# mfinzi/depth-estimation

Hardware: AMD Instinct MI355X
Metric: Mpixel-labels/s per CRF mean-field iter (splat+blur+slice) (higher is better)
Workload: dtype f32; 1 GPU; c3: synthetic 2048x1536x256 cost volume, d=5 bilateral features (BASELINE configs[2]); H=1536, W=2048, L=256, d=5, features=synthetic smooth colours sigma_xy=8.0 sigma_c=0.1, n=3145728, M=296893, parallelism=single GPU, launch=eager, arithmetic=default (fp32-rounding-equivalent, ~1e-7 rel), table=reference

## Files before the change

### depth-estimation_amd/csrc/phl_device_utils.h

```cpp
#pragma once
#include <vector>

#include "phl_internal.h"

namespace {

__device__ __forceinline__ void wave_runs(int key, bool active, int *head_lane, int *run_len)
{
    const int lane = threadIdx.x & 63;
    const int prev = __shfl_up(key, 1);
    const bool prev_active = __shfl_up((int)active, 1) != 0;
    const bool head = active && (lane == 0 || !prev_active || prev != key);
    const unsigned long long heads = __ballot(head);
    const unsigned long long act = __ballot(active);
    const unsigned long long below = heads & ((lane == 63) ? ~0ull : ((2ull << lane) - 1ull));
    *head_lane = 63 - __clzll(below ? below : 1ull);
    const unsigned long long above = (lane == 63) ? 0ull : (heads >> (lane + 1));
    const int next_head = above ? lane + 1 + __ffsll((long long)above) - 1 : 64;
    const int last_active = act ? 64 - __clzll(act) : 0;
    *run_len = min(next_head, last_active) - lane;
}

__device__ __forceinline__ int run_atomic_add(int *counters, int key, bool active)
{
// ... 90 lines not shown

__device__ __forceinline__ void tile_prefix_to_lds(const int *__restrict__ tile_sums, int ntiles, int *pre)
{
    const int b4 = threadIdx.x * 4;
    int v[4], s = 0;
#pragma unroll
    for (int i = 0; i < 4; i++) {
        v[i] = (b4 + i) < ntiles ? tile_sums[b4 + i] : 0;
        s += v[i];
    }
    int tot;
    int ex = block_exclusive_scan(s, &tot);
#pragma unroll
    for (int i = 0; i < 4; i++) {
        pre[b4 + i] = ex;
        ex += v[i];
    }
    __syncthreads();
}

__global__ __launch_bounds__(SCAN_T) void k_scan_add_tiles(int *__restrict__ out, const int *__restrict__ tile_sums, int n)
{
    int s = 0;
    for (int i = threadIdx.x; i < (int)blockIdx.x; i += SCAN_T) s += tile_sums[i];
    int add;
    (void)block_exclusive_scan(s, &add);
    if (blockIdx.x == gridDim.x - 1 && threadIdx.x == 0) out[n] = add + tile_sums[blockIdx.x];
    const int base = blockIdx.x * SCAN_TILE + threadIdx.x * SCAN_I;
#pragma unroll
    for (int i = 0; i < SCAN_I; i++)
        if ((base + i) < n) out[base + i] += add;
}

__attribute__((unused)) int exclusive_scan(const int *in, int *out , int n, int *tile_sums, hipStream_t st)
{
    if (n <= 0) {
        PHL_HIP(hipMemsetAsync(out, 0, sizeof(int), st));
        return PHL_OK;
    }
    const int ntiles = (n + SCAN_TILE - 1) / SCAN_TILE;
    hipLaunchKernelGGL(k_scan_tile, dim3(ntiles), dim3(SCAN_T), 0, st, in, out, tile_sums, n);
    if (ntiles <= SCAN_FUSE_TILES) {
        hipLaunchKernelGGL(k_scan_add_tiles, dim3(ntiles), dim3(SCAN_T), 0, st, out, tile_sums, n);
        PHL_HIP(hipGetLastError());
        return PHL_OK;
    }
    hipLaunchKernelGGL(k_scan_sums, dim3(1), dim3(SCAN_T), 0, st, tile_sums, ntiles, out + n);
    hipLaunchKernelGGL(k_scan_add, dim3(ntiles), dim3(SCAN_T), 0, st, out, tile_sums, n);
    PHL_HIP(hipGetLastError());
    return PHL_OK;
}

struct temp_pool {
    std::vector<void *> ptrs;
    char *base = nullptr;
    size_t cap = 0, off = 0, wanted = 0;
    bool have_cache = false;
    temp_pool() { have_cache = phl_scratch_acquire((void **)&base, &cap); }
    ~temp_pool()
    {
        for (void *p : ptrs) (void)hipFree(p);
        if (have_cache) phl_scratch_release(wanted);
    }
    template <typename T>
    hipError_t get(T **out, size_t count)
    {
        const size_t bytes = (((count ? count : 1) * sizeof(T)) + 255) & ~(size_t)255;
        wanted += bytes;
        if (have_cache && off + bytes <= cap) {
            *out = (T *)(base + off);
            off += bytes;
            return hipSuccess;
        }
        void *p = nullptr;
        hipError_t e = hipMalloc(&p, bytes);
        if (e == hipSuccess) ptrs.push_back(p);
        *out = (T *)p;
        return e;
    }
};

constexpr int RS_TILE = 2048;

// ... 131 lines not shown
```

### depth-estimation_amd/csrc/phl_tiles.hip

```cpp
#include <math.h>
#include <stdio.h>
#include <stdlib.h>

#include <map>
#include <mutex>
#include <type_traits>
#include <utility>
#include <vector>

#include "phl_device_utils.h"

namespace {

__global__ __launch_bounds__(256) void k_minmax(const float *__restrict__ ref, int64_t rs, int64_t cs, int64_t n, int d,
                                                float *__restrict__ out )
{
    __shared__ float smin[4][PHL_MAX_D], smax[4][PHL_MAX_D];
    const int lane = threadIdx.x & 63, w = threadIdx.x >> 6;
    float lo[PHL_MAX_D], hi[PHL_MAX_D];
#pragma unroll
    for (int i = 0; i < PHL_MAX_D; i++) { lo[i] = INFINITY; hi[i] = -INFINITY; }
    for (int64_t p = (int64_t)blockIdx.x * blockDim.x + threadIdx.x; p < n; p += (int64_t)gridDim.x * blockDim.x) {
#pragma unroll
        for (int i = 0; i < PHL_MAX_D; i++)
// ... 421 lines not shown
            carry += __shfl(incl, 63);
        }
    }
    __syncthreads();
    const int64_t vbase = vptr ? (int64_t)vptr[c] : (int64_t)c * stride;
    const int vcap = vptr ? SORTN : stride;
    const int64_t ebase = (int64_t)base * dp1;
    if ((int)threadIdx.x < nv) {
        const int v = threadIdx.x;
        const int ni = atomicAdd(&lbin[256 - min(len, 256)], 1);
        newidx[v] = (unsigned short)ni;
        if (ni < vcap) {
            const int64_t sl = vbase + ni;
            slot_vert[sl] = lvid[v];
            seg_rng[sl] = make_int2((int)(ebase + startv[v]), (int)(ebase + startv[v] + len));
        }
    }
    __syncthreads();
#pragma unroll
    for (int u = 0; u < PER; u++) {
        if (vid[u] < 0) continue;
        const int v = id[u], k = kk[u];
        const int pos = (int)startv[v] + (int)cum[v][k >> 5] + __popc(mask[v * 8 + (k >> 5)] & ((1u << (k & 31)) - 1u));
        phl_contrib_t sg;
        sg.pixel = k;
        sg.w = wgt[u];
        seg[ebase + pos] = sg;
        lidx[ebase + i0 + u] = newidx[v];
    }
}

__global__ __launch_bounds__(256) void k_compact_slots(const int *__restrict__ vptr, int nchunks, int stride,
                                                       const int *__restrict__ t_vert, const int2 *__restrict__ t_rng,
                                                       int *__restrict__ slot_vert, int2 *__restrict__ seg_rng)
{
    const int c = blockIdx.x;
    const int b = vptr[c], nv = vptr[c + 1] - b;
    for (int i = threadIdx.x; i < nv; i += 256) {
        slot_vert[b + i] = t_vert[(int64_t)c * stride + i];
        seg_rng[b + i] = t_rng[(int64_t)c * stride + i];
    }
}

__global__ __launch_bounds__(256) void k_count_slots(const int *__restrict__ slot_vert, int S, int *cnt)
{
    const int s = blockIdx.x * blockDim.x + threadIdx.x;
    if (s < S) atomicAdd(&cnt[slot_vert[s]], 1);
}

__global__ __launch_bounds__(256) void k_contrib_and_sole(const int *__restrict__ perm, int *__restrict__ slot_vert, int S,
                                                          const int *__restrict__ vs_ptr, phl_contrib_t *__restrict__ vs,
                                                          int *__restrict__ multi)
{
    const int s = blockIdx.x * blockDim.x + threadIdx.x;
    if (s >= S) return;
    phl_contrib_t c;
    c.pixel = perm[s];
    c.w = 0.f;
    vs[s] = c;
    const int v = slot_vert[s];
    const bool sole = (vs_ptr[v + 1] - vs_ptr[v]) == 1;
    if (sole) slot_vert[s] = v | (int)0x80000000;
    multi[s] = sole ? 0 : 1;
}

__global__ __launch_bounds__(256) void k_append_long(const int *__restrict__ vs_ptr, int M, int long_list, int *__restrict__ vlong,
                                                     int *__restrict__ count)
{
    const int v = blockIdx.x * blockDim.x + threadIdx.x;
    if (v < M && vs_ptr[v + 1] - vs_ptr[v] > long_list) vlong[atomicAdd(count, 1)] = v;
}

__device__ __forceinline__ float4 ld4(const float *p) { return *reinterpret_cast<const float4 *>(p); }
__device__ __forceinline__ void st4(float *p, float4 v) { *reinterpret_cast<float4 *>(p) = v; }
__device__ __forceinline__ float div_c(float t, float c, float rc)
{
    float q = t * rc;
    float rem = __builtin_fmaf(-q, c, t);
    return __builtin_fmaf(rem, rc, q);
}
__device__ __forceinline__ float4 term4(float4 acc, float w, float4 v, float c, float rc)
{
    return make_float4(acc.x + div_c(w * v.x, c, rc), acc.y + div_c(w * v.y, c, rc), acc.z + div_c(w * v.z, c, rc),
                       acc.w + div_c(w * v.w, c, rc));
}
__device__ __forceinline__ float4 fma4(float4 acc, float w, float4 v)
{
    return make_float4(__builtin_fmaf(w, v.x, acc.x), __builtin_fmaf(w, v.y, acc.y), __builtin_fmaf(w, v.z, acc.z),
                       __builtin_fmaf(w, v.w, acc.w));
}

#define PHL_ROW_BCAST(x, K) ((unsigned)__builtin_amdgcn_update_dpp(0, (int)(x), 0x150 + (K), 0xF, 0xF, false))

template <int K0>
__device__ __forceinline__ float4 sum8(float4 acc, const uint2 e, const char *rbase)
{
    float4 q[8];
    unsigned w[8];
#define PHL_E(k) w[k] = PHL_ROW_BCAST(e.y, K0 + k); q[k] = *reinterpret_cast<const float4 *>(rbase + PHL_ROW_BCAST(e.x, K0 + k));
    PHL_E(0) PHL_E(1) PHL_E(2) PHL_E(3) PHL_E(4) PHL_E(5) PHL_E(6) PHL_E(7)
#undef PHL_E
#pragma unroll
    for (int k = 0; k < 8; k++) acc = fma4(acc, __uint_as_float(w[k]), q[k]);
// ... 742 lines not shown
    const int cnt = min(P, n - base);
    const int E = cnt * dp1;
    const int64_t ebase = (int64_t)base * dp1;
    const int vbase = vptr[c], nv = vptr[c + 1] - vbase;
    uint2 *ent = reinterpret_cast<uint2 *>(lds);
    int *pixl = reinterpret_cast<int *>(ent + P * dp1);
    int *vl = pixl + P;
    const int fixed = (P * dp1 * 8 + P * 4 + nv * 4 + 15) & ~15;
    float *rows = reinterpret_cast<float *>(reinterpret_cast<char *>(lds) + fixed);
    const int mode = fixed + (int64_t)nv * (NS * 128) <= lds_bytes ? 8 : (fixed + (int64_t)nv * (NS * 64) <= lds_bytes ? 4 : 0);
    const unsigned pitch_bytes = (unsigned)NS * (mode == 8 ? 128u : 64u);
    for (int k = threadIdx.x; k < cnt; k += TPB) pixl[k] = pix_order[base + k];
    if (mode)
        for (int i = threadIdx.x; i < nv; i += TPB) vl[i] = slot_vert[vbase + i] & 0x7FFFFFFF;
    for (int e = threadIdx.x; e < E; e += TPB) {
        const int k = e / dp1, r = e - k * dp1;
        const int p = pix_order[base + k];
        const unsigned li = lidx[ebase + e];
        ent[e] = make_uint2(mode ? li * pitch_bytes : (unsigned)(slot_vert[vbase + li] & 0x7FFFFFFF),
                            __float_as_uint(replay[(int64_t)p * dp1 + r].w));
    }
    __syncthreads();
    if (mode == 8)
        slice_grad_chunk<NS, 8, false>(vertw, L, cnt, nv, ent, pixl, vl, rows, y, y_rs, ref, ref_rs, ref_cs, grad_ref, accumulate,
                                       wx_out, wx_rs, rcdiv);
    else if (mode == 4)
        slice_grad_chunk<NS, 4, false>(vertw, L, cnt, nv, ent, pixl, vl, rows, y, y_rs, ref, ref_rs, ref_cs, grad_ref, accumulate,
                                       wx_out, wx_rs, rcdiv);
    else
        slice_grad_chunk<NS, 8, true>(vertw, L, cnt, nv, ent, pixl, vl, rows, y, y_rs, ref, ref_rs, ref_cs, grad_ref, accumulate,
                                      wx_out, wx_rs, rcdiv);
}

__global__ __launch_bounds__(256) void k_fill_vs_rows(phl_contrib_t *__restrict__ vs, int S, const int *__restrict__ slot_pidx)
{
    const int e = blockIdx.x * blockDim.x + threadIdx.x;
    if (e < S) vs[e].w = __int_as_float(slot_pidx[vs[e].pixel]);
}

__global__ __launch_bounds__(256) void k_long_keys(const int *__restrict__ vlong, int n, const int *__restrict__ vs_ptr, int kmax,
                                                   int *__restrict__ key)
{
    const int i = blockIdx.x * blockDim.x + threadIdx.x;
    if (i < n) key[i] = kmax - min(vs_ptr[vlong[i] + 1] - vs_ptr[vlong[i]], kmax);
}

__global__ __launch_bounds__(256) void k_gather_i32(const int *__restrict__ src, const int *__restrict__ perm, int n, int *__restrict__ dst)
{
    const int i = blockIdx.x * blockDim.x + threadIdx.x;
    if (i < n) dst[i] = src[perm[i]];
}

__global__ __launch_bounds__(256) void k_first_slot(const int *__restrict__ slot_vert, int S, const int *__restrict__ vs_ptr,
                                                    const phl_contrib_t *__restrict__ vs, int *__restrict__ first)
{
    const int s = blockIdx.x * blockDim.x + threadIdx.x;
    if (s >= S) return;
    const int v = slot_vert[s] & 0x7FFFFFFF;
    first[s] = (vs[vs_ptr[v]].pixel == s) ? 1 : 0;
}

__global__ __launch_bounds__(256) void k_fill_vorder(const int *__restrict__ slot_vert, int S, const int *__restrict__ first,
                                                     const int *__restrict__ rank, int M_local, int M,
                                                     int *__restrict__ vorder)
{
    const int i = blockIdx.x * blockDim.x + threadIdx.x;
    if (i < S && first[i]) vorder[rank[i]] = slot_vert[i] & 0x7FFFFFFF;
    if (i >= M_local && i < M) vorder[i] = i;
}

__global__ __launch_bounds__(256) void k_strip_marks(int *slot_vert, int S)
{
    const int s = blockIdx.x * blockDim.x + threadIdx.x;
    if (s < S) slot_vert[s] &= 0x7FFFFFFF;
}

template <typename F>
inline void dispatch_lprs(int lprs, F &&f)
{
    switch (lprs) {
        case 64: f(std::integral_constant<int, 64>{}); break;
        case 32: f(std::integral_constant<int, 32>{}); break;
        case 16: f(std::integral_constant<int, 16>{}); break;
        case 8: f(std::integral_constant<int, 8>{}); break;
        default: f(std::integral_constant<int, 4>{}); break;
    }
}

int lds_budget()
{
    static int b = [] {
        const char *e = getenv("PHL_TILE_LDS");
        int v = e ? atoi(e) : 80 * 1024;
        return v < 8192 ? 8192 : (v > 160 * 1024 ? 160 * 1024 : v);
    }();
    return b;
}

inline int64_t lds_extra(int P, int dp1, int nv_max) { return (int64_t)P * dp1 * 8 + (int64_t)P * 4 + ((int64_t)nv_max + 2) * 8 + 16 + 256; }

struct tile_cfg {
    int lprs = -1;
    size_t lds = 0;
    int cap = 0;
};
inline int64_t lds_big() { return lds_budget() > 160 * 1024 ? lds_budget() : 160 * 1024; }

// ... 252 lines not shown
}
fork_slot *fork_from(hipStream_t st)
{
    fork_slot *f = fork_acquire();
    if (f && (hipEventRecord(f->fork, st) != hipSuccess || hipStreamWaitEvent(f->s, f->fork, 0) != hipSuccess)) {
        (void)hipGetLastError();
        fork_release(f);
        f = nullptr;
    }
    return f;
}
struct fork_guard {
    fork_slot *f = nullptr;
    ~fork_guard()
    {
        if (!f) return;
        (void)hipStreamSynchronize(f->s);
        fork_release(f);
    }
    hipError_t join(hipStream_t st)
    {
        if (!f) return hipSuccess;
        hipError_t e = hipEventRecord(f->join, f->s);
        if (e == hipSuccess) e = hipStreamWaitEvent(st, f->join, 0);
        if (e == hipSuccess) {
            fork_release(f);
            f = nullptr;
        }
        return e;
    }
};
}

int phl_tiles_link_vertices(phl_lattice *lat, hipStream_t st)
{
    const int M = (int)lat->M, S = (int)lat->S;
    phl_pinned_reset();
    if (lat->vs_ptr) PHL_HIP(phl_dev_free(lat->vs_ptr));
    if (lat->vs) PHL_HIP(phl_dev_free(lat->vs));
    if (lat->slot_pidx) PHL_HIP(phl_dev_free(lat->slot_pidx));
    lat->vs_ptr = nullptr;
    lat->vs = nullptr;
    lat->slot_pidx = nullptr;
    lat->S_multi = 0;
    PHL_HIP(phl_dev_malloc((void **)&lat->vs_ptr, sizeof(int) * ((size_t)M + 1)));
    PHL_HIP(phl_dev_malloc((void **)&lat->vs, sizeof(phl_contrib_t) * ((size_t)S + 1)));
    PHL_HIP(phl_dev_malloc((void **)&lat->slot_pidx, sizeof(int) * ((size_t)S + 1)));
    if (S == 0) {
        PHL_HIP(hipMemsetAsync(lat->vs_ptr, 0, sizeof(int) * ((size_t)M + 1), st));
        PHL_HIP(hipStreamSynchronize(st));
        return PHL_OK;
    }
    temp_pool tmp;
    int *cnt, *multi, *tile_sums, *sperm;
    PHL_HIP(tmp.get(&cnt, (size_t)M + 1));
    PHL_HIP(tmp.get(&multi, (size_t)S + 1));
    PHL_HIP(tmp.get(&tile_sums, (size_t)(S > M ? S : M) / SCAN_TILE + 2));
    PHL_HIP(tmp.get(&sperm, (size_t)S));
    PHL_HIP(hipMemsetAsync(cnt, 0, sizeof(int) * ((size_t)M + 1), st));
    const unsigned gS = (unsigned)((S + 255) / 256);
    hipLaunchKernelGGL(k_strip_marks, dim3(gS), dim3(256), 0, st, lat->slot_vert, S);
    hipLaunchKernelGGL(k_count_slots, dim3(gS), dim3(256), 0, st, lat->slot_vert, S, cnt);
    PHL_HIP(hipGetLastError());
    int rc = exclusive_scan(cnt, lat->vs_ptr, M, tile_sums, st);
    if (rc) return rc;
    rc = stable_sort_perm(lat->slot_vert, S, M, sperm, tmp, st);
    if (rc) return rc;
    hipLaunchKernelGGL(k_contrib_and_sole, dim3(gS), dim3(256), 0, st, sperm, lat->slot_vert, S, lat->vs_ptr, lat->vs, multi);
    PHL_HIP(hipGetLastError());
    rc = exclusive_scan(multi, lat->slot_pidx, S, tile_sums, st);
    if (rc) return rc;
    hipLaunchKernelGGL(k_fill_vs_rows, dim3(gS), dim3(256), 0, st, lat->vs, S, lat->slot_pidx);
    PHL_HIP(hipGetLastError());
    int pageable_counts[2] = {0, 0};
    int *counts = (int *)phl_pinned_alloc(sizeof(int) * 2);
    if (!counts) counts = pageable_counts;
    PHL_HIP(hipMemcpyAsync(&counts[0], lat->slot_pidx + S, sizeof(int), hipMemcpyDeviceToHost, st));
    int n_long = 0;
    if (lat->vlong) PHL_HIP(phl_dev_free(lat->vlong));
    lat->vlong = nullptr;
    lat->n_long = 0;
    {
        int *lcount;
        PHL_HIP(tmp.get(&lcount, 1));
        PHL_HIP(hipMemsetAsync(lcount, 0, sizeof(int), st));
        PHL_HIP(phl_dev_malloc((void **)&lat->vlong, sizeof(int) * ((size_t)M + 1)));
        hipLaunchKernelGGL(k_append_long, dim3((M + 255) / 256), dim3(256), 0, st, lat->vs_ptr, M, LONG_LIST, lat->vlong, lcount);
        PHL_HIP(hipGetLastError());
        PHL_HIP(hipMemcpyAsync(&counts[1], lcount, sizeof(int), hipMemcpyDeviceToHost, st));
    }
    if (lat->vorder) PHL_HIP(phl_dev_free(lat->vorder));
    lat->vorder = nullptr;
    PHL_HIP(hipStreamSynchronize(st));
    const int s_multi = counts[0];
    n_long = counts[1];
    lat->S_multi = s_multi;
    lat->n_long = n_long;
    if (n_long > 64) {
        int *lkey, *lperm, *lsorted;
        PHL_HIP(tmp.get(&lkey, (size_t)n_long));
        PHL_HIP(tmp.get(&lperm, (size_t)n_long));
        PHL_HIP(tmp.get(&lsorted, (size_t)n_long));
        const unsigned gl = (unsigned)((n_long + 255) / 256);
        const int kmax = lat->nchunks + 1;
        hipLaunchKernelGGL(k_long_keys, dim3(gl), dim3(256), 0, st, lat->vlong, n_long, lat->vs_ptr, kmax, lkey);
        PHL_HIP(hipGetLastError());
        rc = stable_sort_perm(lkey, n_long, (int64_t)kmax + 1, lperm, tmp, st);
        if (rc) return rc;
        hipLaunchKernelGGL(k_gather_i32, dim3(gl), dim3(256), 0, st, lat->vlong, lperm, n_long, lsorted);
        PHL_HIP(hipGetLastError());
        PHL_HIP(hipMemcpyAsync(lat->vlong, lsorted, sizeof(int) * (size_t)n_long, hipMemcpyDeviceToDevice, st));
        PHL_HIP(hipStreamSynchronize(st));
    }
    return PHL_OK;
}

namespace {
int tile_pixels(int dp1)
{
    int P = 2048 / dp1;
    if (P > 256) P = 256;
    P &= ~15;
    if (const char *e = getenv("PHL_TILE_P")) {
        const int v = atoi(e) & ~15;
        if (v >= 16 && v <= P) P = v;
    }
    return P;
}

template <typename Pool>
int pixel_order(phl_lattice *lat, const float *ref, int64_t rs, int64_t cs, int P, const float *lo, const float *hi, int *cell,
                int *nca_out, int *ncb_out, Pool &tmp, hipStream_t st)
{
    const int d = lat->d, n = (int)lat->n;
    int da = 0, db = -1;
    for (int i = 1; i < d; i++)
        if (hi[i] - lo[i] > hi[da] - lo[da]) da = i;
    for (int i = 0; i < d; i++)
        if (i != da && (db < 0 || hi[i] - lo[i] > hi[db] - lo[db])) db = i;
    double ra = (double)hi[da] - lo[da], rb = db >= 0 ? (double)hi[db] - lo[db] : 0.0;
    if (!(ra > 0) || !isfinite(ra)) ra = 0;
    if (!(rb > 0) || !isfinite(rb)) { rb = 0; db = -1; }
    int nca = 1, ncb = 1;
    float inv_t = 0.f;
    if (ra > 0 && n > P) {
        double T = rb > 0 ? sqrt((double)P * ra * rb / n) : (double)P * ra / n;
        if (T > 0 && isfinite(T)) {
// ... 181 lines not shown
    constexpr int SLOT_STRIDE = 384;
    int *t_vert;
    int2 *t_rng;
    PHL_HIP(tmp.get(&t_vert, (size_t)nchunks * SLOT_STRIDE));
    PHL_HIP(tmp.get(&t_rng, (size_t)nchunks * SLOT_STRIDE));
    PHL_HIP(phl_dev_malloc((void **)&lat->seg, sizeof(phl_contrib_t) * (size_t)N));
    PHL_HIP(phl_dev_malloc((void **)&lat->lidx, sizeof(unsigned short) * (size_t)N));
    static const bool use_masks = !(getenv("PHL_CHUNK_MASKS") && atoi(getenv("PHL_CHUNK_MASKS")) == 0);
    if (use_masks) {
        PHL_CHUNK_MASKS(lat->pix_order, n, P, dp1, lat->replay, nv, (const int *)nullptr, SLOT_STRIDE, t_vert, t_rng, lat->seg,
                        lat->lidx)
    } else {
        PHL_CHUNK_SORT(true, lat->pix_order, n, P, dp1, lat->replay, nv, (const int *)nullptr, SLOT_STRIDE, t_vert, t_rng,
                       lat->seg, lat->lidx, (const int *)nullptr, 0)
    }
    PHL_HIP(hipGetLastError());
    rc = exclusive_scan(nv, lat->chunk_vptr, nchunks, tile_sums, st);
    if (rc) return rc;
    std::vector<int> nv_pageable, by_nv_pageable;
    int *nv_host = (int *)phl_pinned_alloc(sizeof(int) * (size_t)nchunks);
    int *by_nv = (int *)phl_pinned_alloc(sizeof(int) * (size_t)nchunks);
    if (!nv_host) { nv_pageable.resize((size_t)nchunks); nv_host = nv_pageable.data(); }
    if (!by_nv) { by_nv_pageable.resize((size_t)nchunks); by_nv = by_nv_pageable.data(); }
    PHL_HIP(hipMemcpyAsync(nv_host, nv, sizeof(int) * (size_t)nchunks, hipMemcpyDeviceToHost, st));
    PHL_HIP(hipStreamSynchronize(st));
    int nv_max = 0;
    for (int c = 0; c < nchunks; c++) {
        const int v = nv_host[c];
        S += v;
        if (v > nv_max) nv_max = v;
    }
    lat->S = S;
    lat->nv_max = nv_max;
    {
        lat->nv_cum = (int *)malloc(sizeof(int) * ((size_t)nv_max + 2));
        if (!lat->nv_cum) { phl_set_error("phl_tiles_build: out of host memory"); return PHL_ERR_HIP; }
        std::vector<int> start((size_t)nv_max + 2, 0);
        for (int c = 0; c < nchunks; c++) start[(size_t)(nv_max - nv_host[c]) + 1]++;
        for (int b = 0; b <= nv_max; b++) start[(size_t)b + 1] += start[(size_t)b];
        for (int x = 0; x <= nv_max; x++) lat->nv_cum[x] = nchunks - start[(size_t)(nv_max - x)];
        for (int c = 0; c < nchunks; c++) by_nv[start[(size_t)(nv_max - nv_host[c])]++] = c;
        PHL_HIP(phl_dev_malloc((void **)&lat->chunk_by_nv, sizeof(int) * ((size_t)nchunks + 1)));
        PHL_HIP(hipMemcpyAsync(lat->chunk_by_nv, by_nv, sizeof(int) * (size_t)nchunks, hipMemcpyHostToDevice, st));
    }
    PHL_HIP(phl_dev_malloc((void **)&lat->slot_vert, sizeof(int) * ((size_t)S + 1)));
    PHL_HIP(phl_dev_malloc((void **)&lat->seg_rng, sizeof(int2) * ((size_t)S + 1)));
    if (nv_max <= SLOT_STRIDE) {
        if (use_masks && nv_max > NVC) {
            PHL_CHUNK_SORT(true, lat->pix_order, n, P, dp1, lat->replay, (int *)nullptr, (const int *)nullptr, SLOT_STRIDE, t_vert,
                           t_rng, lat->seg, lat->lidx, (const int *)nv, NVC)
        }
        hipLaunchKernelGGL(k_compact_slots, dim3(nchunks), dim3(256), 0, st, lat->chunk_vptr, nchunks, SLOT_STRIDE, t_vert,
                           t_rng, lat->slot_vert, lat->seg_rng);
    } else {
        if (use_masks) {
            PHL_CHUNK_MASKS(lat->pix_order, n, P, dp1, lat->replay, (int *)nullptr, lat->chunk_vptr, 0, lat->slot_vert,
                            lat->seg_rng, lat->seg, lat->lidx)
            if (nv_max > NVC) {
                PHL_CHUNK_SORT(true, lat->pix_order, n, P, dp1, lat->replay, (int *)nullptr, lat->chunk_vptr, 0, lat->slot_vert,
                               lat->seg_rng, lat->seg, lat->lidx, (const int *)nv, NVC)
            }
        } else {
            PHL_CHUNK_SORT(true, lat->pix_order, n, P, dp1, lat->replay, (int *)nullptr, lat->chunk_vptr, 0, lat->slot_vert,
                           lat->seg_rng, lat->seg, lat->lidx, (const int *)nullptr, 0)
        }
    }
#undef PHL_CHUNK_SORT
#undef PHL_CHUNK_MASKS
#undef PHL_CHUNK_MASKS_X
    PHL_HIP(hipGetLastError());
    PHL_HIP(nbr_chain.join(st));
    PHL_HIP(hipStreamSynchronize(st));
    }
    phl_release_build_tables(lat);
    rc = phl_tiles_link_vertices(lat, st);
    if (rc) return rc;
    lat->table_bytes = (int64_t)(sizeof(int16_t) * (size_t)lat->M * d + sizeof(phl_replay_t) * (size_t)N +
                                 sizeof(int32_t) * (size_t)lat->M * (d + 1) * 2 + sizeof(int32_t) * (size_t)lat->M * ((d + 1) / 2) * 8 +
                                 sizeof(int) * ((size_t)lat->table_mask + 1) + (lat->int_of_ft ? 2 * sizeof(int) * (size_t)lat->M : 0));
    lat->tile_bytes = (int64_t)(sizeof(int) * ((size_t)n + nchunks + 1 + 3 * ((size_t)S + 1) + (size_t)lat->M + 1) +
                                sizeof(phl_contrib_t) * ((size_t)N + S + 1) + sizeof(unsigned short) * (size_t)N);
    return PHL_OK;
}

int phl_tiles_lprs(const phl_lattice *lat, int vd, int for_slice)
{
    if (lat->nchunks == 0 || vd % 4 != 0) return -1;
    if (for_slice) return 1 << plan_slice(lat, vd).lsh_max;
    return pick_cfg(lat, vd, lat->nv_max).lprs;
}

__global__ __launch_bounds__(256) void k_mark_chunks(const int64_t *__restrict__ rows, int64_t k, const int *__restrict__ vs_ptr,
                                                     const phl_contrib_t *__restrict__ vs, const int *__restrict__ chunk_vptr,
                                                     int nchunks, int *__restrict__ mask)
{
    const int64_t i = (int64_t)blockIdx.x * blockDim.x + threadIdx.x;
    if (i >= k) return;
    const int64_t v = rows[i];
    for (int e = vs_ptr[v]; e < vs_ptr[v + 1]; e++) {
        const int slot = vs[e].pixel;
        int lo = 0, hi = nchunks - 1;
        while (lo < hi) {
            const int mid = (lo + hi + 1) >> 1;
            if (chunk_vptr[mid] <= slot) lo = mid;
            else hi = mid - 1;
        }
        mask[lo] = 1;
    }
}
// ... 5 lines not shown
    temp_pool tmp;
    int *mask;
    PHL_HIP(tmp.get(&mask, (size_t)nchunks));
    PHL_HIP(hipMemsetAsync(mask, 0, sizeof(int) * (size_t)nchunks, st));
    if (k > 0) {
        hipLaunchKernelGGL(k_mark_chunks, dim3((unsigned)((k + 255) / 256)), dim3(256), 0, st, rows_dev, k, lat->vs_ptr, lat->vs,
                           lat->chunk_vptr, nchunks, mask);
        PHL_HIP(hipGetLastError());
    }
    PHL_HIP(hipMemcpyAsync(mask_host, mask, sizeof(int) * (size_t)nchunks, hipMemcpyDeviceToHost, st));
    PHL_HIP(hipStreamSynchronize(st));
    return PHL_OK;
}

int phl_launch_splat_tiled(phl_lattice *lat, const float *src, int64_t src_rs, int vd, float *vert, float *partial,
                           hipStream_t st, bool subset, const int *chunk_list, int nlist, const int *vlist, int64_t nvl,
                           const phl_splat_wide *wide, const int *pack_pos, float *pack, int64_t pack_rs)
{
    if (pack_pos && (!subset || wide)) { phl_set_error("tiled splat: row packing needs a row list and a plain splat"); return PHL_ERR_INVALID; }
    const int64_t out_rs = (int64_t)vd * (wide ? wide->nsets : 1);
    const int M = subset ? (int)nvl : (int)lat->M;
    if (lat->M == 0 || vd == 0) return PHL_OK;
    const tile_plan plan = plan_tiles(lat, vd);
    if (plan.n == 0) {
        phl_set_error("tiled splat: chunk does not fit LDS");
        return PHL_ERR_UNSUPPORTED;
    }
    int rc = PHL_OK;
    const int nrun = subset ? nlist : lat->nchunks;
    static const char *tl_path = getenv("PHL_TIMELINE");
    unsigned long long *tl = nullptr;
    size_t tl_n = 0;
    static const bool side_classes = !(getenv("PHL_SIDE_CLASSES") && atoi(getenv("PHL_SIDE_CLASSES")) == 0);
    fork_slot *fk = (plan.n > 1 && !subset && !tl_path && side_classes) ? fork_from(st) : nullptr;
    hipStream_t const st_main = st;
    int order[12];
    int no = 0;
    for (int ci = 0; ci < plan.n; ci++)
        if (!plan.cls[ci].full_grid) order[no++] = ci;
    for (int ci = 0; ci < plan.n; ci++)
        if (plan.cls[ci].full_grid) order[no++] = ci;
    for (int oi = 0; oi < plan.n && rc == PHL_OK && nrun > 0; oi++) {
        const int ci = fk ? order[oi] : oi;
        const tile_class &c = plan.cls[ci];
        st = (fk && !c.full_grid) ? fk->s : st_main;
        const bool filtered = subset || c.full_grid;
        const int *list = subset ? chunk_list : (c.full_grid ? nullptr : lat->chunk_by_nv + c.begin);
        const int cnt = filtered ? nrun : c.count;
        if (cnt == 0) continue;
        unsigned cgrid;
        int xcd_chunk;
        chunk_grid(cnt, &cgrid, &xcd_chunk);
        unsigned long long *tlc = nullptr;
        if (tl_path && c.full_grid && !tl) {
            tl_n = (size_t)cgrid * 8;
            PHL_HIP(phl_dev_malloc((void **)&tl, tl_n * 8));
            PHL_HIP(hipMemsetAsync(tl, 0, tl_n * 8, st));
            tlc = tl;
        }
        const char *env1 = getenv("PHL_WIDE_ONE_PHASE");
        const bool one_phase = !(env1 && atoi(env1) == 0);
        if (wide && one_phase && c.cfg.lprs == 16 && wide->nsets >= 2 && wide->nsets <= 8 && lat->P <= 256) {
#define PHL_SW(NS_)                                                                                                           \
    case NS_:                                                                                                                 \
        if ((rc = allow_lds(k_splat_wide<NS_>, c.cfg.lds)) != PHL_OK) break;                                                  \
        k_splat_wide<NS_><<<dim3(cgrid), dim3(TPB_S), c.cfg.lds, st>>>(                                                       \
            src, src_rs, vd, (int)lat->n, lat->P, c.cfg.cap, lat->pix_order, lat->chunk_vptr, lat->slot_vert, lat->slot_pidx, \
            lat->seg_rng, lat->seg, vert, partial, cnt, xcd_chunk, list, c.lo, c.hi, long_seg(), wide->fref, wide->rs,        \
            wide->cs);                                                                                                        \
        break;
            switch (wide->nsets) { PHL_SW(2) PHL_SW(3) PHL_SW(4) PHL_SW(5) PHL_SW(6) PHL_SW(7) PHL_SW(8) }
#undef PHL_SW
            continue;
        }
        dispatch_lprs(c.cfg.lprs, [&](auto L) {
            constexpr int LPRS = decltype(L)::value;
            if ((rc = allow_lds(k_splat_tiled<LPRS>, c.cfg.lds)) != PHL_OK) return;
            k_splat_tiled<LPRS><<<dim3(cgrid), dim3(TPB_S), c.cfg.lds, st>>>(
                src, src_rs, vd, (int)lat->n, lat->P, lat->d + 1, c.cfg.cap, lat->pix_order, lat->chunk_vptr, lat->slot_vert,
                lat->slot_pidx, lat->seg_rng, lat->seg, vert, partial, cnt, xcd_chunk, tlc, list, c.lo, c.hi, long_seg(),
                wide ? wide->nsets : 1, wide ? wide->fref : nullptr, wide ? wide->rs : 0, wide ? wide->cs : 0, out_rs);
        });
    }
    st = st_main;
    if (fk) {
        hipError_t e = hipEventRecord(fk->join, fk->s);
        if (e == hipSuccess) e = hipStreamWaitEvent(st, fk->join, 0);
        fork_release(fk);
        if (e != hipSuccess) return phl_hip_fail(e, "joining the side stream of the chunk classes", __FILE__, __LINE__);
    }
    if (tl) {
        std::vector<unsigned long long> h(tl_n);
        PHL_HIP(hipMemcpyAsync(h.data(), tl, tl_n * 8, hipMemcpyDeviceToHost, st));
        PHL_HIP(hipStreamSynchronize(st));
        (void)phl_dev_free(tl);
        if (FILE *f = fopen(tl_path, "wb")) {
            fwrite(h.data(), 8, tl_n, f);
            fclose(f);
        }
    }
    if (rc) return rc;
    if (M == 0) return PHL_OK;
    const int lpr = pick_lpr_row((int)out_rs);
    int64_t waves = ((int64_t)M + (64 / lpr) - 1) / (64 / lpr);
    int64_t blocks = (waves + 3) / 4;
    if (blocks > 2048) blocks = 2048;
    const int *llist = subset ? vlist : lat->vlong;
    const int64_t nl = lat->n_long == 0 ? 0 : (subset ? nvl : lat->n_long);
    const int long_list = llist ? LONG_LIST : 0x7FFFFFFF;
#define PHL_RED(LPR_)                                                                                                  \
    k_splat_reduce<LPR_><<<dim3((unsigned)blocks), dim3(256), 0, st>>>(partial, lat->vs_ptr, lat->vs, lat->slot_pidx, \
                                                                       M, (int)out_rs, vert, vlist, long_list,       \
                                                                       pack_pos, pack, pack_rs);                     \
    if (llist && nl > 0)                                                                                               \
        k_splat_reduce_long<LPR_><<<dim3((unsigned)nl), dim3(256), 0, st>>>(partial, lat->vs_ptr, lat->vs,            \
                                                                            lat->slot_pidx, (int)out_rs, vert, llist, long_list, \
                                                                            subset ? pack_pos : nullptr, pack, pack_rs)
    switch (lpr) {
        case 64: PHL_RED(64); break;
        case 16: PHL_RED(16); break;
        case 4: PHL_RED(4); break;
// ... 79 lines not shown
```

Measured before the change: 367,100 Mpixel-labels/s.

## Replace slot stable sort with counting placement and overlap linking with host build work

Vertex linking no longer uses a stable radix sort. It counts slots per vertex with atomics, places them into per-vertex lists, ranks them within short lists, and orders long lists by chunk using an LDS bitmap. Several small kernels and memsets are merged: zeroing happens inside compact_slots, and the sole/multi marking, long-list append and scan happen in one kernel. Link queueing is split from finishing so the host-side chunk_by_nv construction overlaps GPU work, removing a stream synchronize. This targets lattice build time, which falls outside the per-iteration splat/blur/slice metric, and it adds ordering complexity plus a risk of quadratic cost in the rank loop.

Measured after the change: 367,100 Mpixel-labels/s (median of 2 runs). No clear change (+0.0%).

```diff
diff --git a/depth-estimation_amd/csrc/phl_device_utils.h b/depth-estimation_amd/csrc/phl_device_utils.h
--- a/depth-estimation_amd/csrc/phl_device_utils.h
+++ b/depth-estimation_amd/csrc/phl_device_utils.h
@@ -146,14 +146,9 @@
         if ((base + i) < n) out[base + i] += add;
 }
 
-__attribute__((unused)) int exclusive_scan(const int *in, int *out , int n, int *tile_sums, hipStream_t st)
-{
-    if (n <= 0) {
-        PHL_HIP(hipMemsetAsync(out, 0, sizeof(int), st));
-        return PHL_OK;
-    }
+__attribute__((unused)) int scan_finish(int *out , int n, int *tile_sums, hipStream_t st)
+{
     const int ntiles = (n + SCAN_TILE - 1) / SCAN_TILE;
-    hipLaunchKernelGGL(k_scan_tile, dim3(ntiles), dim3(SCAN_T), 0, st, in, out, tile_sums, n);
     if (ntiles <= SCAN_FUSE_TILES) {
         hipLaunchKernelGGL(k_scan_add_tiles, dim3(ntiles), dim3(SCAN_T), 0, st, out, tile_sums, n);
         PHL_HIP(hipGetLastError());
@@ -163,6 +158,17 @@
     hipLaunchKernelGGL(k_scan_add, dim3(ntiles), dim3(SCAN_T), 0, st, out, tile_sums, n);
     PHL_HIP(hipGetLastError());
     return PHL_OK;
+}
+
+__attribute__((unused)) int exclusive_scan(const int *in, int *out , int n, int *tile_sums, hipStream_t st)
+{
+    if (n <= 0) {
+        PHL_HIP(hipMemsetAsync(out, 0, sizeof(int), st));
+        return PHL_OK;
+    }
+    const int ntiles = (n + SCAN_TILE - 1) / SCAN_TILE;
+    hipLaunchKernelGGL(k_scan_tile, dim3(ntiles), dim3(SCAN_T), 0, st, in, out, tile_sums, n);
+    return scan_finish(out, n, tile_sums, st);
 }
 
 struct temp_pool {
diff --git a/depth-estimation_amd/csrc/phl_tiles.hip b/depth-estimation_amd/csrc/phl_tiles.hip
--- a/depth-estimation_amd/csrc/phl_tiles.hip
+++ b/depth-estimation_amd/csrc/phl_tiles.hip
@@ -477,7 +477,8 @@
 
 __global__ __launch_bounds__(256) void k_compact_slots(const int *__restrict__ vptr, int nchunks, int stride,
                                                        const int *__restrict__ t_vert, const int2 *__restrict__ t_rng,
-                                                       int *__restrict__ slot_vert, int2 *__restrict__ seg_rng)
+                                                       int *__restrict__ slot_vert, int2 *__restrict__ seg_rng,
+                                                       int *__restrict__ zero, int nzero)
 {
     const int c = blockIdx.x;
     const int b = vptr[c], nv = vptr[c + 1] - b;
@@ -485,35 +486,138 @@
         slot_vert[b + i] = t_vert[(int64_t)c * stride + i];
         seg_rng[b + i] = t_rng[(int64_t)c * stride + i];
     }
-}
-
-__global__ __launch_bounds__(256) void k_count_slots(const int *__restrict__ slot_vert, int S, int *cnt)
+    for (int64_t i = (int64_t)blockIdx.x * 256 + threadIdx.x; i < nzero; i += (int64_t)gridDim.x * 256) zero[i] = 0;
+}
+
+__global__ __launch_bounds__(256) void k_count_slots(const int *__restrict__ slot_vert, int S, int *__restrict__ cnt,
+                                                     int *__restrict__ arr)
 {
     const int s = blockIdx.x * blockDim.x + threadIdx.x;
-    if (s < S) atomicAdd(&cnt[slot_vert[s]], 1);
-}
-
-__global__ __launch_bounds__(256) void k_contrib_and_sole(const int *__restrict__ perm, int *__restrict__ slot_vert, int S,
-                                                          const int *__restrict__ vs_ptr, phl_contrib_t *__restrict__ vs,
-                                                          int *__restrict__ multi)
+    if (s < S) arr[s] = atomicAdd(&cnt[slot_vert[s] & 0x7FFFFFFF], 1);
+}
+
+__global__ __launch_bounds__(256) void k_place_slots(const int *__restrict__ slot_vert, int S, const int *__restrict__ vs_ptr,
+                                                     const int *__restrict__ arr, int *__restrict__ lst)
 {
     const int s = blockIdx.x * blockDim.x + threadIdx.x;
-    if (s >= S) return;
-    phl_contrib_t c;
-    c.pixel = perm[s];
-    c.w = 0.f;
-    vs[s] = c;
-    const int v = slot_vert[s];
-    const bool sole = (vs_ptr[v + 1] - vs_ptr[v]) == 1;
-    if (sole) slot_vert[s] = v | (int)0x80000000;
-    multi[s] = sole ? 0 : 1;
-}
-
-__global__ __launch_bounds__(256) void k_append_long(const int *__restrict__ vs_ptr, int M, int long_list, int *__restrict__ vlong,
-                                                     int *__restrict__ count)
-{
-    const int v = blockIdx.x * blockDim.x + threadIdx.x;
-    if (v < M && vs_ptr[v + 1] - vs_ptr[v] > long_list) vlong[atomicAdd(count, 1)] = v;
+    if (s < S) lst[vs_ptr[slot_vert[s] & 0x7FFFFFFF] + arr[s]] = s;
+}
+
+__global__ __launch_bounds__(SCAN_T) void k_rank_mark_scan(int *__restrict__ slot_vert, int S, int M, const int *__restrict__ vs_ptr,
+                                                           const int *__restrict__ lst, int long_list, int *__restrict__ dst,
+                                                           int *__restrict__ slot_pidx, int *__restrict__ tile_sums,
+                                                           int *__restrict__ vlong, int *__restrict__ lcount)
+{
+    const int base = blockIdx.x * SCAN_TILE + threadIdx.x * SCAN_I;
+    int f[SCAN_I], sum = 0;
+#pragma unroll
+    for (int i = 0; i < SCAN_I; i++) {
+        const int s = base + i;
+        f[i] = 0;
+        if (s < S) {
+            const int v = slot_vert[s] & 0x7FFFFFFF;
+            const int b = vs_ptr[v], k = vs_ptr[v + 1] - b;
+            int place = -1;
+            if (k <= long_list) {
+                int r = 0;
+                for (int j = 0; j < k; j++) r += lst[b + j] < s ? 1 : 0;
+                place = b + r;
+            }
+            dst[s] = place;
+            slot_vert[s] = k == 1 ? (v | (int)0x80000000) : v;
+            f[i] = k == 1 ? 0 : 1;
+        }
+        if (s < M && vs_ptr[s + 1] - vs_ptr[s] > long_list) vlong[atomicAdd(lcount, 1)] = s;
+        sum += f[i];
+    }
+    int tot;
+    int ex = block_exclusive_scan(sum, &tot);
+    if (base < S) {
+#pragma unroll
+        for (int i = 0; i < SCAN_I; i++) {
+            if (base + i < S) slot_pidx[base + i] = ex;
+            ex += f[i];
+        }
+    }
+    if (threadIdx.x == 0 && blockIdx.x * SCAN_TILE < S) tile_sums[blockIdx.x] = tot;
+}
+
+constexpr int LONG_BLOCKS = 128, LONG_WIN = 1 << 16;
+__device__ __forceinline__ int chunk_of_slot(const int *__restrict__ vptr, int nchunks, int s)
+{
+    int lo = 0, hi = nchunks - 1;
+    while (lo < hi) {
+        const int mid = (lo + hi + 1) >> 1;
+        if (vptr[mid] <= s) lo = mid;
+        else hi = mid - 1;
+    }
+    return lo;
+}
+
+__global__ __launch_bounds__(256) void k_fill_lists(phl_contrib_t *__restrict__ vs, int S, const int *__restrict__ dst,
+                                                    const int *__restrict__ slot_pidx, int fill_blocks,
+                                                    const int *__restrict__ vs_ptr, const int *__restrict__ lst,
+                                                    const int *__restrict__ vlong, const int *__restrict__ lcount,
+                                                    const int *__restrict__ chunk_vptr, int nchunks, int *__restrict__ counts)
+{
+    if ((int)blockIdx.x < fill_blocks) {
+        const int s = blockIdx.x * 256 + threadIdx.x;
+        if (s == 0) {
+            counts[0] = slot_pidx[S];
+            counts[1] = *lcount;
+        }
+        if (s < S && dst[s] >= 0) {
+            phl_contrib_t c;
+            c.pixel = s;
+            c.w = __int_as_float(slot_pidx[s]);
+            vs[dst[s]] = c;
+        }
+        return;
+    }
+    constexpr int NW = LONG_WIN / 32, WPT = NW / 256;
+    __shared__ unsigned bits[NW];
+    __shared__ int below[NW];
+    const int n_long = *lcount;
+    for (int li = (int)blockIdx.x - fill_blocks; li < n_long; li += LONG_BLOCKS) {
+        const int v = vlong[li];
+        const int b = vs_ptr[v], k = vs_ptr[v + 1] - b;
+        int before = 0;
+        for (int w0 = 0; w0 < nchunks; w0 += LONG_WIN) {
+            for (int w = threadIdx.x; w < NW; w += 256) bits[w] = 0u;
+            __syncthreads();
+            for (int e = threadIdx.x; e < k; e += 256) {
+                const int c = chunk_of_slot(chunk_vptr, nchunks, lst[b + e]) - w0;
+                if (c >= 0 && c < LONG_WIN) atomicOr(&bits[c >> 5], 1u << (c & 31));
+            }
+            __syncthreads();
+            int pc[WPT], sum = 0;
+#pragma unroll
+            for (int i = 0; i < WPT; i++) {
+                pc[i] = __popc(bits[threadIdx.x * WPT + i]);
+                sum += pc[i];
+            }
+            int tot;
+            int ex = block_exclusive_scan(sum, &tot);
+#pragma unroll
+            for (int i = 0; i < WPT; i++) {
+                below[threadIdx.x * WPT + i] = ex;
+                ex += pc[i];
+            }
+            __syncthreads();
+            for (int e = threadIdx.x; e < k; e += 256) {
+                const int s = lst[b + e];
+                const int c = chunk_of_slot(chunk_vptr, nchunks, s) - w0;
+                if (c >= 0 && c < LONG_WIN) {
+                    phl_contrib_t q;
+                    q.pixel = s;
+                    q.w = __int_as_float(slot_pidx[s]);
+                    vs[b + before + below[c >> 5] + __popc(bits[c >> 5] & ((1u << (c & 31)) - 1u))] = q;
+                }
+            }
+            before += tot;
+            __syncthreads();
+        }
+    }
 }
 
 __device__ __forceinline__ float4 ld4(const float *p) { return *reinterpret_cast<const float4 *>(p); }
@@ -1322,12 +1426,6 @@
                                       wx_out, wx_rs, rcdiv);
 }
 
-__global__ __launch_bounds__(256) void k_fill_vs_rows(phl_contrib_t *__restrict__ vs, int S, const int *__restrict__ slot_pidx)
-{
-    const int e = blockIdx.x * blockDim.x + threadIdx.x;
-    if (e < S) vs[e].w = __int_as_float(slot_pidx[vs[e].pixel]);
-}
-
 __global__ __launch_bounds__(256) void k_long_keys(const int *__restrict__ vlong, int n, const int *__restrict__ vs_ptr, int kmax,
                                                    int *__restrict__ key)
 {
@@ -1357,12 +1455,6 @@
     const int i = blockIdx.x * blockDim.x + threadIdx.x;
     if (i < S && first[i]) vorder[rank[i]] = slot_vert[i] & 0x7FFFFFFF;
     if (i >= M_local && i < M) vorder[i] = i;
-}
-
-__global__ __launch_bounds__(256) void k_strip_marks(int *slot_vert, int S)
-{
-    const int s = blockIdx.x * blockDim.x + threadIdx.x;
-    if (s < S) slot_vert[s] &= 0x7FFFFFFF;
 }
 
 template <typename F>
@@ -1681,10 +1773,16 @@
 };
 }
 
-int phl_tiles_link_vertices(phl_lattice *lat, hipStream_t st)
+namespace {
+struct link_pending {
+    int *counts = nullptr;
+    int pageable[2] = {0, 0};
+};
+
+int link_queue(phl_lattice *lat, hipStream_t st, temp_pool &tmp, int *cnt, link_pending *pend)
 {
     const int M = (int)lat->M, S = (int)lat->S;
-    phl_pinned_reset();
+    pend->counts = pend->pageable;
     if (lat->vs_ptr) PHL_HIP(phl_dev_free(lat->vs_ptr));
     if (lat->vs) PHL_HIP(phl_dev_free(lat->vs));
     if (lat->slot_pidx) PHL_HIP(phl_dev_free(lat->slot_pidx));
@@ -1697,53 +1795,50 @@
     PHL_HIP(phl_dev_malloc((void **)&lat->slot_pidx, sizeof(int) * ((size_t)S + 1)));
     if (S == 0) {
         PHL_HIP(hipMemsetAsync(lat->vs_ptr, 0, sizeof(int) * ((size_t)M + 1), st));
-        PHL_HIP(hipStreamSynchronize(st));
+        pend->pageable[1] = lat->n_long;
         return PHL_OK;
     }
-    temp_pool tmp;
-    int *cnt, *multi, *tile_sums, *sperm;
-    PHL_HIP(tmp.get(&cnt, (size_t)M + 1));
-    PHL_HIP(tmp.get(&multi, (size_t)S + 1));
+    if (lat->vlong) PHL_HIP(phl_dev_free(lat->vlong));
+    lat->vlong = nullptr;
+    lat->n_long = 0;
+    PHL_HIP(phl_dev_malloc((void **)&lat->vlong, sizeof(int) * ((size_t)M + 1)));
+    if (lat->vorder) PHL_HIP(phl_dev_free(lat->vorder));
+    lat->vorder = nullptr;
+    int *arr, *lst, *tile_sums, *counts_dev = nullptr;
+    PHL_HIP(tmp.get(&arr, (size_t)S));
+    PHL_HIP(tmp.get(&lst, (size_t)S));
     PHL_HIP(tmp.get(&tile_sums, (size_t)(S > M ? S : M) / SCAN_TILE + 2));
-    PHL_HIP(tmp.get(&sperm, (size_t)S));
-    PHL_HIP(hipMemsetAsync(cnt, 0, sizeof(int) * ((size_t)M + 1), st));
     const unsigned gS = (unsigned)((S + 255) / 256);
-    hipLaunchKernelGGL(k_strip_marks, dim3(gS), dim3(256), 0, st, lat->slot_vert, S);
-    hipLaunchKernelGGL(k_count_slots, dim3(gS), dim3(256), 0, st, lat->slot_vert, S, cnt);
+    if (!cnt) {
+        PHL_HIP(tmp.get(&cnt, (size_t)M + 2));
+        hipLaunchKernelGGL(k_fill_i32, dim3(256), dim3(256), 0, st, cnt, (int64_t)M + 2, 0);
+    }
+    int *lcount = cnt + M + 1;
+    hipLaunchKernelGGL(k_count_slots, dim3(gS), dim3(256), 0, st, lat->slot_vert, S, cnt, arr);
     PHL_HIP(hipGetLastError());
     int rc = exclusive_scan(cnt, lat->vs_ptr, M, tile_sums, st);
     if (rc) return rc;
-    rc = stable_sort_perm(lat->slot_vert, S, M, sperm, tmp, st);
+    hipLaunchKernelGGL(k_place_slots, dim3(gS), dim3(256), 0, st, lat->slot_vert, S, lat->vs_ptr, arr, lst);
+    const int span = S > M ? S : M;
+    hipLaunchKernelGGL(k_rank_mark_scan, dim3((span + SCAN_TILE - 1) / SCAN_TILE), dim3(SCAN_T), 0, st, lat->slot_vert, S, M,
+                       lat->vs_ptr, lst, LONG_LIST, arr, lat->slot_pidx, tile_sums, lat->vlong, lcount);
+    PHL_HIP(hipGetLastError());
+    rc = scan_finish(lat->slot_pidx, S, tile_sums, st);
     if (rc) return rc;
-    hipLaunchKernelGGL(k_contrib_and_sole, dim3(gS), dim3(256), 0, st, sperm, lat->slot_vert, S, lat->vs_ptr, lat->vs, multi);
+    int *counts = (int *)phl_pinned_alloc(sizeof(int) * 2);
+    if (!counts) PHL_HIP(tmp.get(&counts_dev, 2));
+    hipLaunchKernelGGL(k_fill_lists, dim3(gS + LONG_BLOCKS), dim3(256), 0, st, lat->vs, S, arr, lat->slot_pidx, (int)gS,
+                       lat->vs_ptr, lst, lat->vlong, lcount, lat->chunk_vptr, lat->nchunks, counts ? counts : counts_dev);
     PHL_HIP(hipGetLastError());
-    rc = exclusive_scan(multi, lat->slot_pidx, S, tile_sums, st);
-    if (rc) return rc;
-    hipLaunchKernelGGL(k_fill_vs_rows, dim3(gS), dim3(256), 0, st, lat->vs, S, lat->slot_pidx);
-    PHL_HIP(hipGetLastError());
-    int pageable_counts[2] = {0, 0};
-    int *counts = (int *)phl_pinned_alloc(sizeof(int) * 2);
-    if (!counts) counts = pageable_counts;
-    PHL_HIP(hipMemcpyAsync(&counts[0], lat->slot_pidx + S, sizeof(int), hipMemcpyDeviceToHost, st));
-    int n_long = 0;
-    if (lat->vlong) PHL_HIP(phl_dev_free(lat->vlong));
-    lat->vlong = nullptr;
-    lat->n_long = 0;
-    {
-        int *lcount;
-        PHL_HIP(tmp.get(&lcount, 1));
-        PHL_HIP(hipMemsetAsync(lcount, 0, sizeof(int), st));
-        PHL_HIP(phl_dev_malloc((void **)&lat->vlong, sizeof(int) * ((size_t)M + 1)));
-        hipLaunchKernelGGL(k_append_long, dim3((M + 255) / 256), dim3(256), 0, st, lat->vs_ptr, M, LONG_LIST, lat->vlong, lcount);
-        PHL_HIP(hipGetLastError());
-        PHL_HIP(hipMemcpyAsync(&counts[1], lcount, sizeof(int), hipMemcpyDeviceToHost, st));
-    }
-    if (lat->vorder) PHL_HIP(phl_dev_free(lat->vorder));
-    lat->vorder = nullptr;
-    PHL_HIP(hipStreamSynchronize(st));
-    const int s_multi = counts[0];
-    n_long = counts[1];
-    lat->S_multi = s_multi;
+    if (counts) pend->counts = counts;
+    else PHL_HIP(hipMemcpyAsync(pend->pageable, counts_dev, sizeof(int) * 2, hipMemcpyDeviceToHost, st));
+    return PHL_OK;
+}
+
+int link_finish(phl_lattice *lat, hipStream_t st, temp_pool &tmp, const link_pending &pend)
+{
+    const int n_long = pend.counts[1];
+    lat->S_multi = pend.counts[0];
     lat->n_long = n_long;
     if (n_long > 64) {
         int *lkey, *lperm, *lsorted;
@@ -1754,7 +1849,7 @@
         const int kmax = lat->nchunks + 1;
         hipLaunchKernelGGL(k_long_keys, dim3(gl), dim3(256), 0, st, lat->vlong, n_long, lat->vs_ptr, kmax, lkey);
         PHL_HIP(hipGetLastError());
-        rc = stable_sort_perm(lkey, n_long, (int64_t)kmax + 1, lperm, tmp, st);
+        const int rc = stable_sort_perm(lkey, n_long, (int64_t)kmax + 1, lperm, tmp, st);
         if (rc) return rc;
         hipLaunchKernelGGL(k_gather_i32, dim3(gl), dim3(256), 0, st, lat->vlong, lperm, n_long, lsorted);
         PHL_HIP(hipGetLastError());
@@ -1762,6 +1857,19 @@
         PHL_HIP(hipStreamSynchronize(st));
     }
     return PHL_OK;
+}
+}
+
+int phl_tiles_link_vertices(phl_lattice *lat, hipStream_t st)
+{
+    phl_pinned_reset();
+    temp_pool tmp;
+    link_pending pend;
+    const int rc = link_queue(lat, st, tmp, nullptr, &pend);
+    const hipError_t e = hipStreamSynchronize(st);
+    if (rc) return rc;
+    PHL_HIP(e);
+    return link_finish(lat, st, tmp, pend);
 }
 
 namespace {
@@ -2009,26 +2117,20 @@
     }
     lat->S = S;
     lat->nv_max = nv_max;
-    {
-        lat->nv_cum = (int *)malloc(sizeof(int) * ((size_t)nv_max + 2));
-        if (!lat->nv_cum) { phl_set_error("phl_tiles_build: out of host memory"); return PHL_ERR_HIP; }
-        std::vector<int> start((size_t)nv_max + 2, 0);
-        for (int c = 0; c < nchunks; c++) start[(size_t)(nv_max - nv_host[c]) + 1]++;
-        for (int b = 0; b <= nv_max; b++) start[(size_t)b + 1] += start[(size_t)b];
-        for (int x = 0; x <= nv_max; x++) lat->nv_cum[x] = nchunks - start[(size_t)(nv_max - x)];
-        for (int c = 0; c < nchunks; c++) by_nv[start[(size_t)(nv_max - nv_host[c])]++] = c;
-        PHL_HIP(phl_dev_malloc((void **)&lat->chunk_by_nv, sizeof(int) * ((size_t)nchunks + 1)));
-        PHL_HIP(hipMemcpyAsync(lat->chunk_by_nv, by_nv, sizeof(int) * (size_t)nchunks, hipMemcpyHostToDevice, st));
-    }
+    lat->nv_cum = (int *)malloc(sizeof(int) * ((size_t)nv_max + 2));
+    if (!lat->nv_cum) { phl_set_error("phl_tiles_build: out of host memory"); return PHL_ERR_HIP; }
+    PHL_HIP(phl_dev_malloc((void **)&lat->chunk_by_nv, sizeof(int) * ((size_t)nchunks + 1)));
     PHL_HIP(phl_dev_malloc((void **)&lat->slot_vert, sizeof(int) * ((size_t)S + 1)));
     PHL_HIP(phl_dev_malloc((void **)&lat->seg_rng, sizeof(int2) * ((size_t)S + 1)));
+    int *cnt = nullptr;
     if (nv_max <= SLOT_STRIDE) {
         if (use_masks && nv_max > NVC) {
             PHL_CHUNK_SORT(true, lat->pix_order, n, P, dp1, lat->replay, (int *)nullptr, (const int *)nullptr, SLOT_STRIDE, t_vert,
                            t_rng, lat->seg, lat->lidx, (const int *)nv, NVC)
         }
+        PHL_HIP(tmp.get(&cnt, (size_t)lat->M + 2));
         hipLaunchKernelGGL(k_compact_slots, dim3(nchunks), dim3(256), 0, st, lat->chunk_vptr, nchunks, SLOT_STRIDE, t_vert,
-                           t_rng, lat->slot_vert, lat->seg_rng);
+                           t_rng, lat->slot_vert, lat->seg_rng, cnt, (int)lat->M + 2);
     } else {
         if (use_masks) {
             PHL_CHUNK_MASKS(lat->pix_order, n, P, dp1, lat->replay, (int *)nullptr, lat->chunk_vptr, 0, lat->slot_vert,
@@ -2046,12 +2148,28 @@
 #undef PHL_CHUNK_MASKS
 #undef PHL_CHUNK_MASKS_X
     PHL_HIP(hipGetLastError());
-    PHL_HIP(nbr_chain.join(st));
-    PHL_HIP(hipStreamSynchronize(st));
+    link_pending pend;
+    rc = link_queue(lat, st, tmp, cnt, &pend);
+    if (rc) { (void)hipStreamSynchronize(st); return rc; }
+    {
+        std::vector<int> start((size_t)nv_max + 2, 0);
+        for (int c = 0; c < nchunks; c++) start[(size_t)(nv_max - nv_host[c]) + 1]++;
+        for (int b = 0; b <= nv_max; b++) start[(size_t)b + 1] += start[(size_t)b];
+        for (int x = 0; x <= nv_max; x++) lat->nv_cum[x] = nchunks - start[(size_t)(nv_max - x)];
+        for (int c = 0; c < nchunks; c++) by_nv[start[(size_t)(nv_max - nv_host[c])]++] = c;
+        const hipError_t e = hipMemcpyAsync(lat->chunk_by_nv, by_nv, sizeof(int) * (size_t)nchunks, hipMemcpyHostToDevice, st);
+        if (e != hipSuccess) { (void)hipStreamSynchronize(st); PHL_HIP(e); }
+    }
+    {
+        const hipError_t e = nbr_chain.join(st);
+        const hipError_t e2 = hipStreamSynchronize(st);
+        PHL_HIP(e);
+        PHL_HIP(e2);
+    }
+    rc = link_finish(lat, st, tmp, pend);
+    if (rc) { (void)hipStreamSynchronize(st); return rc; }
     }
     phl_release_build_tables(lat);
-    rc = phl_tiles_link_vertices(lat, st);
-    if (rc) return rc;
     lat->table_bytes = (int64_t)(sizeof(int16_t) * (size_t)lat->M * d + sizeof(phl_replay_t) * (size_t)N +
                                  sizeof(int32_t) * (size_t)lat->M * (d + 1) * 2 + sizeof(int32_t) * (size_t)lat->M * ((d + 1) / 2) * 8 +
                                  sizeof(int) * ((size_t)lat->table_mask + 1) + (lat->int_of_ft ? 2 * sizeof(int) * (size_t)lat->M : 0));
@@ -2123,7 +2241,9 @@
     unsigned long long *tl = nullptr;
     size_t tl_n = 0;
     static const bool side_classes = !(getenv("PHL_SIDE_CLASSES") && atoi(getenv("PHL_SIDE_CLASSES")) == 0);
-    fork_slot *fk = (plan.n > 1 && !subset && !tl_path && side_classes) ? fork_from(st) : nullptr;
+    fork_guard side;
+    if (plan.n > 1 && !subset && !tl_path && side_classes) side.f = fork_from(st);
+    fork_slot *const fk = side.f;
     hipStream_t const st_main = st;
     int order[12];
     int no = 0;
@@ -2175,9 +2295,7 @@
     }
     st = st_main;
     if (fk) {
-        hipError_t e = hipEventRecord(fk->join, fk->s);
-        if (e == hipSuccess) e = hipStreamWaitEvent(st, fk->join, 0);
-        fork_release(fk);
+        const hipError_t e = side.join(st);
         if (e != hipSuccess) return phl_hip_fail(e, "joining the side stream of the chunk classes", __FILE__, __LINE__);
     }
     if (tl) {
```
